# alibaba/EasyRec

Hardware: NVIDIA H100
Metric: samples_per_sec (higher is better)
Workload: dtype f32

## Files before the change

easyrec_b200/_lib.py:

```python
import ctypes
import os

import numpy as np

_HERE = os.path.dirname(os.path.abspath(__file__))
LIB_PATH = os.environ.get('ER_LIB_PATH') or os.path.join(_HERE, 'lib', 'liber_b200.so')

c_i32, c_i64, c_f32 = ctypes.c_int32, ctypes.c_int64, ctypes.c_float
c_vp, c_sz = ctypes.c_void_p, ctypes.c_size_t

SLOT_DTYPE = np.dtype(
    [('num_buckets', '<i8'), ('row_offset', '<i8'), ('seg_begin', '<i4'),
     ('n_seg', '<i4'), ('bucket_mode', '<i4'), ('combiner', '<i4'),
     ('out_buf', '<i4'), ('out_stride', '<i4'), ('out_col', '<i4'),
     ('shard_n', '<i4')],
    align=True)
assert SLOT_DTYPE.itemsize == 48
DENSE_SEG_DTYPE = np.dtype([('offset', '<i8'), ('n', '<i8'), ('l2', '<f4'), ('lr_mult', '<f4')], align=True)
assert DENSE_SEG_DTYPE.itemsize == 24

BUCKET_FARM_DECIMAL, BUCKET_MOD, BUCKET_IDENTITY, BUCKET_NONE, BUCKET_ONE_ROW = 0, 1, 2, 3, 4
COMBINER_SUM, COMBINER_MEAN, COMBINER_SQRTN = 0, 1, 2
COMBINER_UNIT_WEIGHTS = 16
OPT_SGD, OPT_ADAGRAD, OPT_LAZY_ADAM, OPT_ADAM_ROWS, OPT_MOMENTUM = 0, 1, 2, 3, 4
ACT_GELU, ACT_LEAKY_RELU, ACT_ELU, ACT_SELU, ACT_TANH, ACT_SWISH, ACT_SIGMOID = 1, 2, 3, 4, 5, 6, 7
MAX_BUFS = 8
ABI_VERSION = 3
HYPER_LR, HYPER_BETA1_POWER, HYPER_BETA2_POWER, HYPER_GRAD_SCALE, HYPER_N = 0, 1, 2, 3, 4


class ErOpt(ctypes.Structure):
  _fields_ = [('kind', c_i32), ('lr', c_f32), ('beta1', c_f32),
              ('beta2', c_f32), ('eps', c_f32), ('beta1_power', c_f32),
              ('beta2_power', c_f32), ('grad_scale', c_f32), ('hyper_dev', c_vp)]


class ErBnStats(ctypes.Structure):
  _fields_ = [('bias', c_vp), ('save_mean', c_vp), ('save_rstd', c_vp), ('moving_mean', c_vp),
              ('moving_var', c_vp), ('eps', c_f32), ('momentum', c_f32)]


class ErCsvCol(ctypes.Structure):
  _fields_ = [('kind', c_i32), ('width', c_i32), ('inner_sep', ctypes.c_char), ('kv_sep', ctypes.c_char), ('pad_', ctypes.c_char * 6),
              ('default_i64', c_i64), ('default_f32', c_f32), ('pad2_', c_i32), ('default_str', ctypes.c_char_p),
              ('out', c_vp), ('lens', c_vp), ('list_cap', c_i64), ('n_vals', c_i64), ('hash_mod', ctypes.c_uint64), ('weights', c_vp),
              ('step_lens', c_vp)]


ER_OK, ER_ERR_INVALID_ARG, ER_ERR_WORKSPACE, ER_ERR_CUDA, ER_ERR_UNSUPPORTED = range(5)
CSV_SKIP, CSV_I64, CSV_F32, CSV_HASH, CSV_I64_LIST, CSV_F32_VEC, CSV_HASH_LIST, CSV_I64_KV_LIST, CSV_HASH_KV_LIST, CSV_F32_LIST, \
    CSV_I64_STEP_LIST, CSV_HASH_STEP_LIST = range(12)

SIGNATURES = {
    'er_abi_version': (c_i32, []),
# ... 64 lines not shown
    'er_split_cols': (c_i32, [c_vp, c_i32, c_i64, ctypes.POINTER(c_vp), ctypes.POINTER(c_i32),
                              ctypes.POINTER(c_i32), c_i32, c_vp]),
    'er_rowsum_block_fwd': (c_i32, [c_vp, c_i64, c_i32, c_i32, c_vp, c_vp, c_vp, c_sz, c_vp]),
    'er_rowsum_block_bwd': (c_i32, [c_vp, c_vp, c_vp, c_f32, c_i64, c_i32, c_i32, c_vp, c_i32, c_vp]),
    'er_dense1_workspace_bytes': (c_sz, [c_i32]),
    'er_dense1_fwd': (c_i32, [c_vp, c_vp, c_vp, c_i64, c_i32, c_i32, c_vp, c_vp]),
    'er_dense1_bwd': (c_i32, [c_vp, c_vp, c_vp, c_i64, c_i32, c_i32, c_vp, c_i32, c_vp, c_vp, c_vp, c_sz, c_vp]),
    'er_gemm_bn_workspace_bytes': (c_sz, [c_i64, c_i64]),
    'er_gemm_bn': (c_i32, [c_vp, c_i64, c_i32, c_vp, c_i64, c_i32, c_vp, c_i64, c_i64, c_i64, c_i64,
                           ctypes.POINTER(ErBnStats), c_vp, c_sz, c_vp]),
    'er_bn_act_apply': (c_i32, [c_vp, c_vp, c_vp, c_vp, c_vp, c_vp, c_i64, c_i32, c_i32, c_vp, c_vp]),
    'er_fm_block_workspace_bytes': (c_sz, [c_i64]),
    'er_fm_block_fwd': (c_i32, [c_vp, c_i64, c_i32, c_i32, c_i32, c_vp, c_vp, c_vp, c_sz, c_vp]),
    'er_fm_block_bwd': (c_i32, [c_vp, c_vp, c_vp, c_vp, c_f32, c_i64, c_i32, c_i32, c_i32, c_i32, c_vp, c_i32,
                                c_vp]),
    'er_gemm_workspace_bytes': (c_sz, [c_i64, c_i64, c_i64]),
    'er_gemm': (c_i32, [c_vp, c_i64, c_i32, c_vp, c_i64, c_i32, c_vp, c_vp, c_i64, c_i64, c_i64, c_i64,
                        c_vp, c_sz, c_vp]),
    'er_bias_bn_act_fwd': (c_i32, [c_vp, c_vp, c_vp, c_vp, c_vp, c_vp, c_i64,
                                   c_i32, c_f32, c_f32, c_i32, c_i32, c_vp,
                                   c_vp, c_vp, c_vp, c_sz, c_vp]),
    'er_bias_bn_act_bwd': (c_i32, [c_vp, c_vp, c_vp, c_vp, c_vp, c_vp, c_vp,
                                   c_i64, c_i32, c_i32, c_vp, c_vp, c_vp, c_vp,
                                   c_vp, c_sz, c_vp]),
    'er_din_concat_fwd': (c_i32, [c_vp, c_vp, c_i64, c_i32, c_i32, c_vp, c_vp]),
    'er_din_concat_bwd': (c_i32, [c_vp, c_vp, c_vp, c_i64, c_i32, c_i32, c_vp, c_vp, c_i32, c_vp]),
    'er_din_pool_fwd': (c_i32, [c_vp, c_vp, c_vp, c_i64, c_i32, c_i32, c_vp, c_vp, c_vp]),
    'er_din_pool_bwd': (c_i32, [c_vp, c_vp, c_vp, c_vp, c_i64, c_i32, c_i32, c_vp, c_vp, c_i32, c_vp]),
    'er_din_sigmoid_pool_fwd': (c_i32, [c_vp, c_vp, c_vp, c_i64, c_i32, c_i32, c_f32, c_vp, c_vp, c_vp]),
    'er_din_sigmoid_pool_bwd': (c_i32, [c_vp, c_vp, c_vp, c_vp, c_i64, c_i32, c_i32, c_f32, c_vp, c_vp, c_i32,
# ... 54 lines not shown
```

easyrec_b200/csrc/gemm.cu:

```cuda
#include <algorithm>

#include "common.cuh"

namespace er {
namespace gemm {

constexpr int BM = 128, BN = 128, BK = 32;
constexpr int kStages = 3;
constexpr int kPrefetch = 2;
constexpr int kThreads = 256;
constexpr int kTileBytes = 128 * 128;
constexpr int kStageBytes = 4 * kTileBytes;
constexpr int kOutPitch = BN + 8;
constexpr int kStatFloats = 768;
constexpr int kSmemBytes = kStages * kStageBytes + 1024  + kStatFloats * 4 + 16;
static_assert(BM * kOutPitch * 4 <= kStages * kStageBytes, "output tile must fit in the stage ring");

struct Args {
  const float* A;
  const float* B;
  float* C;
  const float* bias;
  float* partials;
  long long lda, ldb, ldc;
  int M, N, K;
  int a_mn, b_mn;
  int k_per_slice;
  int n_slices;
  float* bn_part;
  unsigned int* bn_counter;
  er_bn_stats_t bn;
};

__device__ __forceinline__ uint32_t smem_u32(const void* p) {
  return static_cast<uint32_t>(__cvta_generic_to_shared(p));
}

__device__ __forceinline__ uint64_t make_desc(uint32_t smem_addr) {
  uint64_t d = 0;
  d |= (uint64_t)((smem_addr >> 4) & 0x3fff);
  d |= (uint64_t)1 << 16;
  d |= (uint64_t)(1024 >> 4) << 32;
  d |= (uint64_t)1 << 62;
  return d;
}

__device__ __forceinline__ void wgmma_fence() { asm volatile("wgmma.fence.sync.aligned;" ::: "memory"); }
__device__ __forceinline__ void wgmma_commit() { asm volatile("wgmma.commit_group.sync.aligned;" ::: "memory"); }
template <int N>
__device__ __forceinline__ void wgmma_wait() {
// ... 45 lines not shown
      "%16, %17, %18, %19, %20, %21, %22, %23, %24, %25, %26, %27, %28, %29, %30, %31, "
      "%32, %33, %34, %35, %36, %37, %38, %39, %40, %41, %42, %43, %44, %45, %46, %47, "
      "%48, %49, %50, %51, %52, %53, %54, %55, %56, %57, %58, %59, %60, %61, %62, %63"
      "}, %64, %65, p, 1, 1;\n}\n"
      : "+f"(d[0]), "+f"(d[1]), "+f"(d[2]), "+f"(d[3]), "+f"(d[4]), "+f"(d[5]), "+f"(d[6]), "+f"(d[7]),
        "+f"(d[8]), "+f"(d[9]), "+f"(d[10]), "+f"(d[11]), "+f"(d[12]), "+f"(d[13]), "+f"(d[14]), "+f"(d[15]),
        "+f"(d[16]), "+f"(d[17]), "+f"(d[18]), "+f"(d[19]), "+f"(d[20]), "+f"(d[21]), "+f"(d[22]), "+f"(d[23]),
        "+f"(d[24]), "+f"(d[25]), "+f"(d[26]), "+f"(d[27]), "+f"(d[28]), "+f"(d[29]), "+f"(d[30]), "+f"(d[31]),
        "+f"(d[32]), "+f"(d[33]), "+f"(d[34]), "+f"(d[35]), "+f"(d[36]), "+f"(d[37]), "+f"(d[38]), "+f"(d[39]),
        "+f"(d[40]), "+f"(d[41]), "+f"(d[42]), "+f"(d[43]), "+f"(d[44]), "+f"(d[45]), "+f"(d[46]), "+f"(d[47]),
        "+f"(d[48]), "+f"(d[49]), "+f"(d[50]), "+f"(d[51]), "+f"(d[52]), "+f"(d[53]), "+f"(d[54]), "+f"(d[55]),
        "+f"(d[56]), "+f"(d[57]), "+f"(d[58]), "+f"(d[59]), "+f"(d[60]), "+f"(d[61]), "+f"(d[62]), "+f"(d[63])
      : "l"(da), "l"(db), "r"(1));
}

__device__ __forceinline__ void split_tf32(float x, float& hi, float& lo) {
  uint32_t h = (__float_as_uint(x) + 0x1000u) & 0xffffe000u;
  hi = __uint_as_float(h);
  lo = x - hi;
}

__device__ __forceinline__ float4 mask_chunk(float4 v, int nvalid) {
  if (nvalid < 4) {
    if (nvalid < 1) v.x = 0.f;
    if (nvalid < 2) v.y = 0.f;
    if (nvalid < 3) v.z = 0.f;
    v.w = 0.f;
  }
  return v;
}

struct Pos {
  int mn, k;
};
__device__ __forceinline__ Pos pos_of(int mn_major, int warp, int lane, int j) {
  if (!mn_major) return Pos{(lane >> 3) + 4 * warp + 32 * j, 4 * (lane & 7)};
// ... 35 lines not shown
  }
}

struct Welford {
  float n, mean, m2;
};
__device__ __forceinline__ void wf_merge(Welford& a, const Welford& b) {
  if (b.n == 0.f) return;
  const float n = a.n + b.n;
  const float d = b.mean - a.mean;
  a.mean += d * (b.n / n);
  a.m2 += b.m2 + d * d * (a.n * b.n / n);
  a.n = n;
}

template <int NM>
__global__ void __launch_bounds__(kThreads, 1) gemm_tf32x3_kernel(Args a) {
  constexpr int R = NM / 2;
  extern __shared__ uint8_t smem_raw[];
  const uint32_t raw_u32 = smem_u32(smem_raw);
  const uint32_t smem_base = (raw_u32 + 1023u) & ~1023u;
  uint8_t* base_ptr = smem_raw + (smem_base - raw_u32);
  float* s_stats = reinterpret_cast<float*>(base_ptr + kStages * kStageBytes);
  int* s_flag = reinterpret_cast<int*>(s_stats + kStatFloats);

  const int tid = threadIdx.x, warp = tid >> 5, lane = tid & 31, wg = warp >> 2;
  const int n0 = blockIdx.x * BN, m0 = blockIdx.y * BM;
  const int k_begin = blockIdx.z * a.k_per_slice;
  const int k_end = min(a.K, k_begin + a.k_per_slice);
  const int n_kb = (k_end - k_begin + BK - 1) / BK;

  Pos pa[4], pb[4];
#pragma unroll
  for (int j = 0; j < 4; ++j) {
    pa[j] = pos_of(a.a_mn, warp, lane, j);
    pb[j] = pos_of(a.b_mn, warp, lane, j);
  }
  float4 va[kPrefetch][4], vb[kPrefetch][4];
  auto issue = [&](int kb, float4 (&xa)[4], float4 (&xb)[4]) {
    const int k0 = k_begin + kb * BK;
#pragma unroll
    for (int j = 0; j < 4; ++j) {
      xa[j] = load_pos(a.A, a.lda, a.a_mn, pa[j], m0, a.M, k0, k_end);
      xb[j] = pb[j].mn < NM ? load_pos(a.B, a.ldb, a.b_mn, pb[j], n0, a.N, k0, k_end)
                            : make_float4(0.f, 0.f, 0.f, 0.f);
    }
  };
  auto stage_out = [&](int kb, const float4 (&xa)[4], const float4 (&xb)[4]) {
    const int k0 = k_begin + kb * BK;
    const uint32_t st = smem_base + (uint32_t)(kb % kStages) * kStageBytes;
#pragma unroll
    for (int j = 0; j < 4; ++j) {
      store_pos(st, a.a_mn, pa[j], mask_chunk(xa[j], pos_nvalid(a.a_mn, pa[j], m0, a.M, k0, k_end)));
      if (pb[j].mn < NM)
        store_pos(st + 2 * kTileBytes, a.b_mn, pb[j], mask_chunk(xb[j], pos_nvalid(a.b_mn, pb[j], n0, a.N, k0, k_end)));
    }
  };

  float acc[R], acc2[R];
#pragma unroll
  for (int i = 0; i < R; ++i) acc[i] = acc2[i] = 0.f;

  er_pdl_wait();
#pragma unroll
  for (int u = 0; u < kPrefetch; ++u)
    if (u < n_kb) issue(u, va[u], vb[u]);

  for (int kb0 = 0; kb0 < n_kb; kb0 += kPrefetch) {
#pragma unroll
    for (int u = 0; u < kPrefetch; ++u) {
      const int kb = kb0 + u;
      if (kb < n_kb) {
        stage_out(kb, va[u], vb[u]);
        if (kb + kPrefetch < n_kb) issue(kb + kPrefetch, va[u], vb[u]);
        asm volatile("fence.proxy.async.shared::cta;" ::: "memory");
        __syncthreads();
        const uint32_t st = smem_base + (uint32_t)(kb % kStages) * kStageBytes;
        const uint32_t a_hi = st + (uint32_t)wg * (64u * 128u), b_hi = st + 2 * kTileBytes;
        fence_regs(acc);
        fence_regs(acc2);
        wgmma_fence();
#pragma unroll
        for (int kk = 0; kk < BK / 8; ++kk) {
          const uint64_t ahi = make_desc(a_hi + kk * 32), alo = make_desc(a_hi + kTileBytes + kk * 32);
          const uint64_t bhi = make_desc(b_hi + kk * 32), blo = make_desc(b_hi + kTileBytes + kk * 32);
          wgmma_tf32(acc2, alo, bhi);
          wgmma_tf32(acc2, ahi, blo);
          wgmma_tf32(acc, ahi, bhi);
        }
        wgmma_commit();
        wgmma_wait<1>();
// ... 146 lines not shown

static void plan(int64_t M, int64_t N, int64_t K, int* n_slices, int* k_per_slice) {
  const int64_t tiles = ceil_div(M, BM) * ceil_div(N, BN);
  const int64_t kblocks = ceil_div(K, BK);
  int64_t s = 1;
  if (tiles * 2 <= kSmCount && kblocks >= 16) {
    s = kSmCount / tiles;
    s = std::min<int64_t>(s, kblocks / 8);
    s = std::max<int64_t>(s, 1);
  }
  const int64_t per = ceil_div(kblocks, s);
  *k_per_slice = (int)(per * BK);
  *n_slices = (int)ceil_div(kblocks, per);
}

template <int NM>
static int launch(const Args& a, dim3 grid, cudaStream_t st) {
  static bool attr_set = false;
  if (!attr_set) {
    cudaError_t e = cudaFuncSetAttribute(gemm_tf32x3_kernel<NM>, cudaFuncAttributeMaxDynamicSharedMemorySize,
                                         kSmemBytes);
    if (e != cudaSuccess) return er::fail(ER_ERR_CUDA, std::string("er_gemm: ") + cudaGetErrorString(e));
    attr_set = true;
  }
  er::launch_pdl(gemm_tf32x3_kernel<NM>, grid, dim3(kThreads), (size_t)kSmemBytes, st, a);
  return ER_OK;
}

}
}

extern "C" size_t er_gemm_workspace_bytes(int64_t M, int64_t N, int64_t K) {
  int s, kp;
  er::gemm::plan(M, N, K, &s, &kp);
  return s > 1 ? (size_t)s * (size_t)M * (size_t)N * sizeof(float) : 0;
}

extern "C" size_t er_gemm_bn_workspace_bytes(int64_t M, int64_t N);

static int gemm_impl(const float* A, int64_t lda, int32_t a_mn_major, const float* B, int64_t ldb,
                     int32_t b_mn_major, const float* bias, float* C, int64_t ldc, int64_t M, int64_t N,
                     int64_t K, const er_bn_stats_t* bn, void* ws, size_t ws_bytes, er_stream_t stream) {
  using namespace er::gemm;
  ER_REQUIRE(A && B && C, "null operand");
  ER_REQUIRE(M > 0 && N > 0 && K > 0 && M < (1ll << 31) && N < (1ll << 31) && K < (1ll << 31), "bad shape");
  ER_REQUIRE((lda & 3) == 0 && (ldb & 3) == 0, "operand pitch must be a multiple of 4 floats");
  ER_REQUIRE((reinterpret_cast<uintptr_t>(A) & 15) == 0 && (reinterpret_cast<uintptr_t>(B) & 15) == 0,
             "operands must be 16-byte aligned");
  ER_REQUIRE(lda >= (a_mn_major ? M : K) && ldb >= (b_mn_major ? N : K), "pitch smaller than row");
  ER_REQUIRE(ldc >= N, "ldc < N");
  Args a;
  a.A = A; a.B = B; a.C = C; a.bias = bias;
  a.lda = lda; a.ldb = ldb; a.ldc = ldc;
  a.M = (int)M; a.N = (int)N; a.K = (int)K;
  a.a_mn = a_mn_major ? 1 : 0; a.b_mn = b_mn_major ? 1 : 0;
  plan(M, N, K, &a.n_slices, &a.k_per_slice);
  a.partials = nullptr;
  a.bn_part = nullptr;
  a.bn_counter = nullptr;
  if (a.n_slices > 1) {
    ER_REQUIRE(!bn, "batch-norm statistics need an unsplit K (er_gemm_workspace_bytes(M,N,K) == 0)");
    ER_REQUIRE(ws && ws_bytes >= er_gemm_workspace_bytes(M, N, K), "workspace too small");
    a.partials = static_cast<float*>(ws);
  }
  if (bn) {
    ER_REQUIRE(bn->save_mean && bn->save_rstd, "bn: save_mean / save_rstd missing");
    ER_REQUIRE((bn->moving_mean == nullptr) == (bn->moving_var == nullptr), "bn: moving_mean and moving_var go together");
    ER_REQUIRE(ws && ws_bytes >= er_gemm_bn_workspace_bytes(M, N), "bn workspace too small");
    a.bn = *bn;
    a.bn_counter = static_cast<unsigned int*>(ws);
    a.bn_part = reinterpret_cast<float*>(static_cast<char*>(ws) + 1024);
  }
  cudaStream_t st = er::as_stream(stream);
  dim3 grid((unsigned)er::ceil_div(N, BN), (unsigned)er::ceil_div(M, BM), (unsigned)a.n_slices);
  const int rc = N > 64 ? launch<128>(a, grid, st) : N > 32 ? launch<64>(a, grid, st)
               : N > 16 ? launch<32>(a, grid, st) : launch<16>(a, grid, st);
  if (rc != ER_OK) return rc;
  int launches = 1;
  if (a.n_slices > 1) {
    const long long total = (long long)M * N;
    int blocks = (int)std::min<long long>((total + 255) / 256, 4LL * er::kSmCount);
    er::launch_pdl(splitk_reduce_kernel, dim3(blocks), dim3(256), 0, st, (const float*)a.partials, bias, C,
                   (long long)ldc, (int)M, (int)N, a.n_slices);
    ++launches;
  }
  er::count_launches(launches);
  ER_CUDA_LAUNCH_CHECK();
  return ER_OK;
}

extern "C" int er_gemm(const float* A, int64_t lda, int32_t a_mn_major, const float* B, int64_t ldb,
                       int32_t b_mn_major, const float* bias, float* C, int64_t ldc, int64_t M, int64_t N,
                       int64_t K, void* ws, size_t ws_bytes, er_stream_t stream) {
  return gemm_impl(A, lda, a_mn_major, B, ldb, b_mn_major, bias, C, ldc, M, N, K, nullptr, ws, ws_bytes, stream);
}

extern "C" size_t er_gemm_bn_workspace_bytes(int64_t M, int64_t N) {
  return 1024 + (size_t)er::ceil_div(M, er::gemm::BM) * (size_t)N * 3 * sizeof(float);
}

extern "C" int er_gemm_bn(const float* A, int64_t lda, int32_t a_mn_major, const float* B, int64_t ldb,
                          int32_t b_mn_major, float* C, int64_t ldc, int64_t M, int64_t N, int64_t K,
                          const er_bn_stats_t* bn, void* ws, size_t ws_bytes, er_stream_t stream) {
  if (!bn) return er::fail(ER_ERR_INVALID_ARG, "er_gemm_bn: bn is NULL");
  if (er::ceil_div(N, er::gemm::BN) > 256) return er::fail(ER_ERR_INVALID_ARG, "er_gemm_bn: N too large");
  return gemm_impl(A, lda, a_mn_major, B, ldb, b_mn_major, nullptr, C, ldc, M, N, K, bn, ws, ws_bytes, stream);
}
```

easyrec_b200/kernels.py:

```python
import ctypes

import numpy as np
import torch

from easyrec_b200 import _lib
from easyrec_b200._lib import ErOpt, SLOT_DTYPE, c_vp


def _stream():
  return torch.cuda.current_stream().cuda_stream


def _p(t):
  return None if t is None else t.data_ptr()


def _chk(t, dtype, name):
  if t is None:
    return
  if not t.is_cuda:
    raise _lib.ErError('%s must be a CUDA tensor (no CPU fallback)' % name)
  if t.dtype != dtype:
    raise _lib.ErError('%s must be %s, got %s' % (name, dtype, t.dtype))
  if not t.is_contiguous():
# ... 507 lines not shown
      buf = torch.zeros(t.shape[0], (t.shape[1] + 3) // 4 * 4, dtype=torch.float32, device=t.device)
      buf[:, :t.shape[1]].copy_(t)
      t = buf[:, :t.shape[1]]
    else:
      t = t.contiguous() if not t.is_contiguous() else t.clone()
  raise ValueError('%s: cannot be laid out for er_gemm' % name)


def gemm_ready(t):
  return _gemm_operand(t, 'x')[0]


_gemm_ws = {}


def gemm(a, b, bias=None, out=None):
  lib = _lib.load()
  M, Ka = a.shape
  Kb, N = b.shape
  assert Ka == Kb, (a.shape, b.shape)
  if N < 8 or Ka < 8 or M < 8:
    return gemm_small(a, b, bias, out)
  a, lda, a_unit = _gemm_operand(a, 'a')
  b, ldb, b_unit = _gemm_operand(b, 'b')
  if out is None:
    out = torch.empty(M, N, dtype=torch.float32, device=a.device)
  assert out.stride(1) == 1
  nbytes = lib.er_gemm_workspace_bytes(M, N, Ka)
  ws = None
  if nbytes:
    key = (a.device, torch.cuda.current_stream().cuda_stream if a.is_cuda else 0)
    ws = _gemm_ws.get(key)
    if ws is None or ws.numel() < nbytes:
      ws = torch.empty(nbytes, dtype=torch.uint8, device=a.device)
      _gemm_ws[key] = ws
  _lib.check(lib.er_gemm(_p(a), lda, 0 if a_unit else 1, _p(b), ldb, 1 if b_unit else 0, _p(bias), _p(out),
                         out.stride(0), M, N, Ka, _p(ws), 0 if ws is None else ws.numel(), _stream()), 'er_gemm')
  return out


def gemm_small(a, b, bias=None, out=None):
  lib = _lib.load()
  M, Ka = a.shape
  _, N = b.shape
  for t, name in ((a, 'a'), (b, 'b')):
    if not t.is_cuda or t.dtype != torch.float32:
      raise _lib.ErError('%s must be a CUDA fp32 matrix (no CPU fallback)' % name)
  _chk(bias, torch.float32, 'bias')
  if out is None:
    out = torch.empty(M, N, dtype=torch.float32, device=a.device)
# ... 3 lines not shown
  if nbytes:
    key = (a.device, torch.cuda.current_stream().cuda_stream, 'small')
    ws = _gemm_ws.get(key)
    if ws is None or ws.numel() < nbytes:
      ws = torch.empty(nbytes, dtype=torch.uint8, device=a.device)
      _gemm_ws[key] = ws
  _lib.check(lib.er_gemm_small(_p(a), a.stride(0), a.stride(1), _p(b), b.stride(0), b.stride(1), _p(bias), _p(out),
                               out.stride(0), M, N, Ka, _p(ws), 0 if ws is None else ws.numel(), _stream()),
             'er_gemm_small')
  return out


_gemm_bn_ws = {}


def gemm_bn(a, b, bias, moving_mean, moving_var, eps, momentum):
  lib = _lib.load()
  M, Ka = a.shape
  Kb, N = b.shape
  assert Ka == Kb, (a.shape, b.shape)
  if N < 8 or Ka < 8 or M < 8 or lib.er_gemm_workspace_bytes(M, N, Ka) != 0:
    return None
  a, lda, a_unit = _gemm_operand(a, 'a')
  b, ldb, b_unit = _gemm_operand(b, 'b')
  z = torch.empty(M, N, dtype=torch.float32, device=a.device)
  mean = torch.empty(N, dtype=torch.float32, device=a.device)
  rstd = torch.empty(N, dtype=torch.float32, device=a.device)
  nbytes = lib.er_gemm_bn_workspace_bytes(M, N)
  key = (a.device, torch.cuda.current_stream().cuda_stream if a.is_cuda else 0)
  ws = _gemm_bn_ws.get(key)
  if ws is None or ws.numel() < nbytes:
    ws = torch.zeros(nbytes, dtype=torch.uint8, device=a.device)
    _gemm_bn_ws[key] = ws
  bn = _lib.ErBnStats(_p(bias), _p(mean), _p(rstd), _p(moving_mean), _p(moving_var), eps, momentum)
  _lib.check(lib.er_gemm_bn(_p(a), lda, 0 if a_unit else 1, _p(b), ldb, 1 if b_unit else 0, _p(z), z.stride(0),
                            M, N, Ka, ctypes.byref(bn), _p(ws), ws.numel(), _stream()), 'er_gemm_bn')
  return z, mean, rstd


def bn_act_apply(z, bias, gamma, beta, mean, rstd, relu, y=None):
  lib = _lib.load()
  _chk(z, torch.float32, 'z')
  batch, units = z.shape
  if y is None:
    y = torch.empty_like(z)
  _lib.check(lib.er_bn_act_apply(_p(z), _p(bias), _p(gamma), _p(beta), _p(mean), _p(rstd), batch, units,
                                 1 if relu else 0, _p(y), _stream()), 'er_bn_act_apply')
  return y


def dense_workspace(batch, units, device):
  lib = _lib.load()
# ... 35 lines not shown
```

easyrec_b200/layers.py:

```python
import math
import os

import torch
from torch import nn

from easyrec_b200 import kernels as K

BN_EPS = 1e-3
BN_MOMENTUM = 0.99
_OVERLAP_DW_DX = os.environ.get('ER_OVERLAP_DW_DX', '1') == '1'
_side = {}
_defer = {'on': False, 'dirty': set()}


class defer_dw_join(object):

  def __enter__(self):
    self.prev = _defer['on']
    _defer['on'] = True
    return self

  def __exit__(self, *exc):
    _defer['on'] = self.prev
    if not self.prev:
      for dev in list(_defer['dirty']):
        torch.cuda.current_stream(dev).wait_stream(_side[dev])
      _defer['dirty'].clear()
    return False


def _side_stream(device):
  s = _side.get(device)
  if s is None:
    s = torch.cuda.Stream(device=device)
    _side[device] = s
  return s


class _DenseBNAct(torch.autograd.Function):

  @staticmethod
  def forward(ctx, x, kernel, bias, gamma, beta, moving_mean, moving_var, training, relu, ws):
    x = K.gemm_ready(x)
    ctx.kernel_param = kernel
    if hasattr(kernel, '_er_uses'):
      kernel._er_uses += 1
    fused = None
    if gamma is not None and training:
      fused = K.gemm_bn(x, kernel, bias, moving_mean, moving_var, BN_EPS, BN_MOMENTUM)
    if fused is not None:
      z, mean, rstd = fused
      y = K.bn_act_apply(z, bias, gamma, beta, mean, rstd, relu)
    else:
      z = K.gemm(x, kernel)
      y, mean, rstd = K.bias_bn_act_fwd(z, bias, gamma, beta, moving_mean, moving_var, BN_EPS,
                                        BN_MOMENTUM, training, relu, ws)
    ctx.relu = relu
    ctx.ws = ws
    ctx.has_bn = gamma is not None
    ctx.save_for_backward(x, kernel, bias, gamma, z, y, mean, rstd)
    return y

  @staticmethod
  def backward(ctx, gy):
    x, kernel, bias, gamma, z, y, mean, rstd = ctx.saved_tensors
    gz, gbias, ggamma, gbeta = K.bias_bn_act_bwd(z, bias, gamma, y, gy.contiguous(), mean, rstd,
                                                 ctx.relu, ctx.ws)
    kp = ctx.kernel_param
    dst = getattr(kp, '_er_grad_out', None)
    if dst is not None and getattr(kp, '_er_uses', 2) == 1 and kp.grad is None:
      gk = dst.view_as(dst)
    else:
      gk = torch.empty(x.shape[1], gz.shape[1], dtype=torch.float32, device=x.device)
    if ctx.needs_input_grad[0] and x.is_cuda and _OVERLAP_DW_DX:
      cur = torch.cuda.current_stream()
      side = _side_stream(x.device)
      side.wait_stream(cur)
      with torch.cuda.stream(side):
        K.gemm(x.t(), gz, out=gk)
      gx = K.gemm(gz, kernel.t())
      if _defer['on']:
        gz.record_stream(side)
        x.record_stream(side)
        _defer['dirty'].add(x.device)
      else:
        cur.wait_stream(side)
    else:
      K.gemm(x.t(), gz, out=gk)
      gx = K.gemm(gz, kernel.t()) if ctx.needs_input_grad[0] else None
    return gx, gk, gbias, ggamma, gbeta, None, None, None, None, None


class _Dense1(torch.autograd.Function):

  @staticmethod
  def forward(ctx, x, kernel, bias):
    if x.stride(1) != 1:
      x = x.contiguous()
    ctx.save_for_backward(x, kernel)
    return K.dense1_fwd(x, kernel, bias)

  @staticmethod
  def backward(ctx, gy):
    x, kernel = ctx.saved_tensors
# ... 278 lines not shown
```

easyrec_b200/trainer.py:

```python
import ctypes

import numpy as np
import torch

from easyrec_b200 import _lib
from easyrec_b200 import kernels as K
from easyrec_b200 import layers as L


class FlatDenseOptimizer(object):

  def __init__(self, named_params, kind, lr, l2_of=None, beta1=0.9, beta2=0.999, eps=1e-8,
               adagrad_init=0.1):
    self.names = [n for n, _ in named_params]
    self.params = [p for _, p in named_params]
    dev = self.params[0].device
    sizes = [p.numel() for p in self.params]
    self.sizes = sizes
    total = sum((n + 3) // 4 * 4 for n in sizes)
    self.flat_p = torch.zeros(total, dtype=torch.float32, device=dev)
    self.flat_g = torch.zeros(total, dtype=torch.float32, device=dev)
    off = 0
    segs = np.zeros(len(sizes), dtype=_lib.DENSE_SEG_DTYPE)
    self.grad_views = []
# ... 116 lines not shown
class Trainer(object):

  def __init__(self, model, input_layer, dense_optimizer='adagrad', lr=0.01, lr_fn=None,
               use_cuda_graph=False, world_size=1, beta1=0.9, beta2=0.999, adagrad_init=0.1, dense_lr_fn=None,
               dense_betas=None, clip_norm=0.0):
    self.model = model
    self.input_layer = input_layer
    self.lr = lr
    self.lr_fn = lr_fn or (lambda step: lr)
    named = [(n, p) for n, p in model.named_parameters() if p.requires_grad]
    l2 = getattr(model, 'l2_of', None)
    db1, db2 = dense_betas or (beta1, beta2)
    self.dense_opt = FlatDenseOptimizer(named, dense_optimizer, lr, l2_of=l2, beta1=db1, beta2=db2,
                                        adagrad_init=adagrad_init)
    self.beta1, self.beta2 = beta1, beta2
    self.dense_lr_fn = dense_lr_fn
    if dense_lr_fn is None:
      self.dense_opt.hyper = input_layer.hyper
    self.world = world_size
    self.clip_norm = float(clip_norm or 0.0)
    self.last_grad_norm = None
    self.dp = None
    if world_size > 1:
      from easyrec_b200.distributed import DataParallel
      ep = bool(getattr(input_layer, 'ep', False))
      if self.clip_norm and ep:
        input_layer.ep_hold_updates(True)
      self.dp = DataParallel(input_layer, self.dense_opt, world_size, sparse=not ep)
    dev = str(getattr(input_layer, 'device', 'cpu'))
    self._ep_side = torch.cuda.Stream(device=dev) if (self.dp is not None and not self.dp.sparse and
# ... 8 lines not shown
    self._warm_stream = None
    self._graph = None
    self._step_pending = []
    self._static = None
    self._loss = None
    self._probs = None

  def _set_hyper(self):
    lr = self.lr_fn(self.step)
    self.input_layer.set_optimizer_step(lr, self.step, beta1=self.beta1, beta2=self.beta2)
    if self.dense_lr_fn is not None:
      self.dense_opt.hyper.set(self.dense_lr_fn(self.step), self.step)

  def _segment_compute(self, features, labels, next_features=None):
    self.dense_opt.zero_grad()
    logits = self.model(features)
    if next_features is not None:
      self.input_layer.prefetch_exchange(next_features)
    sw = features.get('sample_weight') if isinstance(features, dict) else None
    if sw is not None:
      loss, probs = self.model.loss(logits, labels, sample_weight=sw)
    else:
      loss, probs = self.model.loss(logits, labels)
    with L.defer_dw_join():
      loss.backward()
    self.dense_opt.gather_grads()
    self._step_pending = list(self.input_layer._pending)
    return loss.detach(), probs

  def _segment_exchange(self):
    if self.dp is not None:
      if not self.dp.sparse:
        if self._ep_side is not None:
          self._ep_side.wait_stream(torch.cuda.current_stream())
        with torch.cuda.stream(self._ep_side):
          self.input_layer.backward_update()
      self.dp.exchange(self._step_pending)
      self.dp.join_presort()

  def _clip_by_global_norm(self):
# ... 109 lines not shown
```

include/er_b200.h:

```cpp
#ifndef ER_B200_H_
#define ER_B200_H_

#include <stddef.h>
#include <stdint.h>

#ifdef __cplusplus
extern "C" {
#endif

#define ER_B200_ABI_VERSION 3

typedef void* er_stream_t;

typedef enum er_status {
  ER_OK = 0,
  ER_ERR_INVALID_ARG = 1,
  ER_ERR_WORKSPACE = 2,
  ER_ERR_CUDA = 3,
  ER_ERR_UNSUPPORTED = 4
} er_status;

typedef enum er_bucket_mode {
  ER_BUCKET_FARM_DECIMAL = 0,
  ER_BUCKET_MOD = 1,
// ... 228 lines not shown
                  er_stream_t stream);

typedef struct {
  const float* bias;
  float* save_mean;
  float* save_rstd;
  float* moving_mean;
  float* moving_var;
  float eps;
  float momentum;
} er_bn_stats_t;
size_t er_gemm_bn_workspace_bytes(int64_t M, int64_t N);
int er_gemm_bn(const float* A, int64_t lda, int32_t a_mn_major, const float* B, int64_t ldb,
               int32_t b_mn_major, float* C, int64_t ldc, int64_t M, int64_t N, int64_t K,
               const er_bn_stats_t* bn, void* ws, size_t ws_bytes, er_stream_t stream);
int er_bn_act_apply(const float* z, const float* bias, const float* gamma, const float* beta,
                    const float* mean, const float* rstd, int64_t batch, int32_t units, int32_t relu,
                    float* y, er_stream_t stream);

int er_sigmoid_ce_fwd_bwd(const float* logits, const float* labels,
                          const float* weights, int64_t batch, float inv_count,
                          float* loss_out, float* probs, float* g_logits,
                          er_stream_t stream);

int er_din_concat_fwd(const float* query, const float* keys, int64_t batch,
                      int32_t seq_len, int32_t dim, float* din_in, er_stream_t stream);
int er_din_concat_bwd(const float* query, const float* keys, const float* g_din_in,
                      int64_t batch, int32_t seq_len, int32_t dim, float* g_query,
                      float* g_keys, int32_t accumulate_gkeys, er_stream_t stream);
int er_din_pool_fwd(const float* scores, const float* keys, const int32_t* lens,
// ... 87 lines not shown
```

Before: 9.935 million.

## Pre-split dense weights into swizzled TF32 hi/lo planes loaded by bulk copy

Once per step, a batched kernel splits each dense tower weight (and its transpose) into TF32 hi/lo planes laid out in the GEMM's swizzled shared-memory tile format. Forward and dX GEMMs then fetch the B operand with cp.async.bulk on mbarriers instead of per-thread loads, splitting and storing. This removes repeated per-CTA B splitting and register staging, and frees registers to deepen A prefetch. It costs an extra split kernel and plane memory every step, and adds mbarrier synchronisation complexity.

```diff
diff --git a/easyrec_b200/_lib.py b/easyrec_b200/_lib.py
--- a/easyrec_b200/_lib.py
+++ b/easyrec_b200/_lib.py
@@ -38,6 +38,11 @@
 class ErBnStats(ctypes.Structure):
   _fields_ = [('bias', c_vp), ('save_mean', c_vp), ('save_rstd', c_vp), ('moving_mean', c_vp),
               ('moving_var', c_vp), ('eps', c_f32), ('momentum', c_f32)]
+
+
+class ErGemmPlane(ctypes.Structure):
+  _fields_ = [('src', c_vp), ('ld_row', c_i64), ('ld_k', c_i64), ('rows', c_i64), ('k', c_i64), ('hi', c_vp),
+              ('lo', c_vp)]
 
 
 class ErCsvCol(ctypes.Structure):
@@ -132,6 +137,10 @@
     'er_fm_block_fwd': (c_i32, [c_vp, c_i64, c_i32, c_i32, c_i32, c_vp, c_vp, c_vp, c_sz, c_vp]),
     'er_fm_block_bwd': (c_i32, [c_vp, c_vp, c_vp, c_vp, c_f32, c_i64, c_i32, c_i32, c_i32, c_i32, c_vp, c_i32,
                                 c_vp]),
+    'er_gemm_plane_floats': (c_sz, [c_i64, c_i64]),
+    'er_gemm_split_planes': (c_i32, [ctypes.POINTER(ErGemmPlane), c_i32, c_vp]),
+    'er_gemm_planes': (c_i32, [c_vp, c_i64, c_i32, c_vp, c_vp, c_vp, c_vp, c_i64, c_i64, c_i64, c_i64,
+                               ctypes.POINTER(ErBnStats), c_vp, c_sz, c_vp]),
     'er_gemm_workspace_bytes': (c_sz, [c_i64, c_i64, c_i64]),
     'er_gemm': (c_i32, [c_vp, c_i64, c_i32, c_vp, c_i64, c_i32, c_vp, c_vp, c_i64, c_i64, c_i64, c_i64,
                         c_vp, c_sz, c_vp]),
diff --git a/easyrec_b200/csrc/gemm.cu b/easyrec_b200/csrc/gemm.cu
--- a/easyrec_b200/csrc/gemm.cu
+++ b/easyrec_b200/csrc/gemm.cu
@@ -1,6 +1,7 @@
 #include <algorithm>
 
 #include "common.cuh"
+#include "tf32_split.cuh"
 
 namespace er {
 namespace gemm {
@@ -8,12 +9,13 @@
 constexpr int BM = 128, BN = 128, BK = 32;
 constexpr int kStages = 3;
 constexpr int kPrefetch = 2;
+constexpr int kPrefetchPre = 3;
 constexpr int kThreads = 256;
 constexpr int kTileBytes = 128 * 128;
 constexpr int kStageBytes = 4 * kTileBytes;
 constexpr int kOutPitch = BN + 8;
 constexpr int kStatFloats = 768;
-constexpr int kSmemBytes = kStages * kStageBytes + 1024  + kStatFloats * 4 + 16;
+constexpr int kSmemBytes = kStages * kStageBytes + 1024  + kStatFloats * 4 + 16 + kStages * 8;
 static_assert(BM * kOutPitch * 4 <= kStages * kStageBytes, "output tile must fit in the stage ring");
 
 struct Args {
@@ -25,6 +27,9 @@
   long long lda, ldb, ldc;
   int M, N, K;
   int a_mn, b_mn;
+  const float* b_hi;
+  const float* b_lo;
+  long long b_tile_floats;
   int k_per_slice;
   int n_slices;
   float* bn_part;
@@ -32,8 +37,30 @@
   er_bn_stats_t bn;
 };
 
+__host__ __device__ constexpr int mma_width(long long n) { return n > 64 ? 128 : n > 32 ? 64 : n > 16 ? 32 : 16; }
+__host__ __device__ constexpr long long plane_tile_floats(long long rows, long long k) {
+  return (k + BK - 1) / BK * mma_width(rows) * BK;
+}
+
 __device__ __forceinline__ uint32_t smem_u32(const void* p) {
   return static_cast<uint32_t>(__cvta_generic_to_shared(p));
+}
+
+__device__ __forceinline__ void mbar_init(uint32_t bar, uint32_t count) {
+  asm volatile("mbarrier.init.shared::cta.b64 [%0], %1;" ::"r"(bar), "r"(count) : "memory");
+}
+__device__ __forceinline__ void mbar_expect_tx(uint32_t bar, uint32_t bytes) {
+  asm volatile("mbarrier.arrive.expect_tx.shared::cta.b64 _, [%0], %1;" ::"r"(bar), "r"(bytes) : "memory");
+}
+__device__ __forceinline__ void mbar_wait(uint32_t bar, uint32_t parity) {
+  asm volatile(
+      "{\n.reg .pred p;\nWAIT_%=:\n"
+      "mbarrier.try_wait.parity.shared::cta.b64 p, [%0], %1;\n"
+      "@!p bra WAIT_%=;\n}\n" ::"r"(bar), "r"(parity) : "memory");
+}
+__device__ __forceinline__ void bulk_g2s(uint32_t dst, const void* src, uint32_t bytes, uint32_t bar) {
+  asm volatile("cp.async.bulk.shared::cluster.global.mbarrier::complete_tx::bytes [%0], [%1], %2, [%3];"
+               ::"r"(dst), "l"(src), "r"(bytes), "r"(bar) : "memory");
 }
 
 __device__ __forceinline__ uint64_t make_desc(uint32_t smem_addr) {
@@ -109,12 +136,6 @@
       : "l"(da), "l"(db), "r"(1));
 }
 
-__device__ __forceinline__ void split_tf32(float x, float& hi, float& lo) {
-  uint32_t h = (__float_as_uint(x) + 0x1000u) & 0xffffe000u;
-  hi = __uint_as_float(h);
-  lo = x - hi;
-}
-
 __device__ __forceinline__ float4 mask_chunk(float4 v, int nvalid) {
   if (nvalid < 4) {
     if (nvalid < 1) v.x = 0.f;
@@ -180,15 +201,17 @@
   a.n = n;
 }
 
-template <int NM>
+template <int NM, bool kPreB>
 __global__ void __launch_bounds__(kThreads, 1) gemm_tf32x3_kernel(Args a) {
   constexpr int R = NM / 2;
+  constexpr int kPf = kPreB ? kPrefetchPre : kPrefetch;
   extern __shared__ uint8_t smem_raw[];
   const uint32_t raw_u32 = smem_u32(smem_raw);
   const uint32_t smem_base = (raw_u32 + 1023u) & ~1023u;
   uint8_t* base_ptr = smem_raw + (smem_base - raw_u32);
   float* s_stats = reinterpret_cast<float*>(base_ptr + kStages * kStageBytes);
   int* s_flag = reinterpret_cast<int*>(s_stats + kStatFloats);
+  const uint32_t s_bar = smem_u32(s_flag + 4);
 
   const int tid = threadIdx.x, warp = tid >> 5, lane = tid & 31, wg = warp >> 2;
   const int n0 = blockIdx.x * BN, m0 = blockIdx.y * BM;
@@ -202,14 +225,15 @@
     pa[j] = pos_of(a.a_mn, warp, lane, j);
     pb[j] = pos_of(a.b_mn, warp, lane, j);
   }
-  float4 va[kPrefetch][4], vb[kPrefetch][4];
+  float4 va[kPf][4], vb[kPreB ? 1 : kPf][4];
   auto issue = [&](int kb, float4 (&xa)[4], float4 (&xb)[4]) {
     const int k0 = k_begin + kb * BK;
 #pragma unroll
     for (int j = 0; j < 4; ++j) {
       xa[j] = load_pos(a.A, a.lda, a.a_mn, pa[j], m0, a.M, k0, k_end);
-      xb[j] = pb[j].mn < NM ? load_pos(a.B, a.ldb, a.b_mn, pb[j], n0, a.N, k0, k_end)
-                            : make_float4(0.f, 0.f, 0.f, 0.f);
+      if constexpr (!kPreB)
+        xb[j] = pb[j].mn < NM ? load_pos(a.B, a.ldb, a.b_mn, pb[j], n0, a.N, k0, k_end)
+                              : make_float4(0.f, 0.f, 0.f, 0.f);
     }
   };
   auto stage_out = [&](int kb, const float4 (&xa)[4], const float4 (&xb)[4]) {
@@ -218,29 +242,50 @@
 #pragma unroll
     for (int j = 0; j < 4; ++j) {
       store_pos(st, a.a_mn, pa[j], mask_chunk(xa[j], pos_nvalid(a.a_mn, pa[j], m0, a.M, k0, k_end)));
-      if (pb[j].mn < NM)
+      if (!kPreB && pb[j].mn < NM)
         store_pos(st + 2 * kTileBytes, a.b_mn, pb[j], mask_chunk(xb[j], pos_nvalid(a.b_mn, pb[j], n0, a.N, k0, k_end)));
     }
   };
+  auto issue_b = [&](int kb) {
+    constexpr uint32_t kPlaneBytes = NM * BK * 4;
+    const uint32_t st = smem_base + (uint32_t)(kb % kStages) * kStageBytes + 2 * kTileBytes;
+    const uint32_t bar = s_bar + 8u * (uint32_t)(kb % kStages);
+    const long long off = (long long)blockIdx.x * a.b_tile_floats + (long long)(k_begin / BK + kb) * (NM * BK);
+    mbar_expect_tx(bar, 2 * kPlaneBytes);
+    bulk_g2s(st, a.b_hi + off, kPlaneBytes, bar);
+    bulk_g2s(st + kTileBytes, a.b_lo + off, kPlaneBytes, bar);
+  };
+  if constexpr (kPreB) {
+    if (tid == 0) {
+      for (int s = 0; s < kStages; ++s) mbar_init(s_bar + 8u * s, 1);
+      asm volatile("fence.mbarrier_init.release.cluster;" ::: "memory");
+    }
+    __syncthreads();
+  }
 
   float acc[R], acc2[R];
 #pragma unroll
   for (int i = 0; i < R; ++i) acc[i] = acc2[i] = 0.f;
 
   er_pdl_wait();
-#pragma unroll
-  for (int u = 0; u < kPrefetch; ++u)
-    if (u < n_kb) issue(u, va[u], vb[u]);
-
-  for (int kb0 = 0; kb0 < n_kb; kb0 += kPrefetch) {
-#pragma unroll
-    for (int u = 0; u < kPrefetch; ++u) {
+  if (kPreB && tid == 0 && n_kb > 0) issue_b(0);
+#pragma unroll
+  for (int u = 0; u < kPf; ++u)
+    if (u < n_kb) issue(u, va[u], vb[kPreB ? 0 : u]);
+
+  for (int kb0 = 0; kb0 < n_kb; kb0 += kPf) {
+#pragma unroll
+    for (int u = 0; u < kPf; ++u) {
       const int kb = kb0 + u;
       if (kb < n_kb) {
-        stage_out(kb, va[u], vb[u]);
-        if (kb + kPrefetch < n_kb) issue(kb + kPrefetch, va[u], vb[u]);
+        stage_out(kb, va[u], vb[kPreB ? 0 : u]);
+        if (kb + kPf < n_kb) issue(kb + kPf, va[u], vb[kPreB ? 0 : u]);
         asm volatile("fence.proxy.async.shared::cta;" ::: "memory");
         __syncthreads();
+        if constexpr (kPreB) {
+          if (tid == 0 && kb + 1 < n_kb) issue_b(kb + 1);
+          mbar_wait(s_bar + 8u * (uint32_t)(kb % kStages), (uint32_t)(kb / kStages) & 1u);
+        }
         const uint32_t st = smem_base + (uint32_t)(kb % kStages) * kStageBytes;
         const uint32_t a_hi = st + (uint32_t)wg * (64u * 128u), b_hi = st + 2 * kTileBytes;
         fence_regs(acc);
@@ -417,17 +462,53 @@
   *n_slices = (int)ceil_div(kblocks, per);
 }
 
-template <int NM>
+template <int NM, bool kPreB>
 static int launch(const Args& a, dim3 grid, cudaStream_t st) {
   static bool attr_set = false;
   if (!attr_set) {
-    cudaError_t e = cudaFuncSetAttribute(gemm_tf32x3_kernel<NM>, cudaFuncAttributeMaxDynamicSharedMemorySize,
+    cudaError_t e = cudaFuncSetAttribute(gemm_tf32x3_kernel<NM, kPreB>, cudaFuncAttributeMaxDynamicSharedMemorySize,
                                          kSmemBytes);
     if (e != cudaSuccess) return er::fail(ER_ERR_CUDA, std::string("er_gemm: ") + cudaGetErrorString(e));
     attr_set = true;
   }
-  er::launch_pdl(gemm_tf32x3_kernel<NM>, grid, dim3(kThreads), (size_t)kSmemBytes, st, a);
+  er::launch_pdl(gemm_tf32x3_kernel<NM, kPreB>, grid, dim3(kThreads), (size_t)kSmemBytes, st, a);
   return ER_OK;
+}
+template <bool kPreB>
+static int launch_width(const Args& a, dim3 grid, cudaStream_t st) {
+  switch (mma_width(a.N)) {
+    case 128: return launch<128, kPreB>(a, grid, st);
+    case 64: return launch<64, kPreB>(a, grid, st);
+    case 32: return launch<32, kPreB>(a, grid, st);
+    default: return launch<16, kPreB>(a, grid, st);
+  }
+}
+
+constexpr int kMaxPlaneJobs = 32;
+struct PlaneJobs {
+  er_gemm_plane_t j[kMaxPlaneJobs];
+};
+__global__ void split_planes_kernel(PlaneJobs jobs) {
+  const er_gemm_plane_t p = jobs.j[blockIdx.y];
+  const int nm = mma_width(p.rows);
+  const long long n_kb = (p.k + BK - 1) / BK;
+  const long long chunks = (p.rows + BN - 1) / BN * n_kb * nm * (BK / 4);
+  er_pdl_wait();
+  for (long long i = (long long)blockIdx.x * blockDim.x + threadIdx.x; i < chunks; i += (long long)gridDim.x * blockDim.x) {
+    const int c = (int)(i & 7);
+    const long long rk = i >> 3;
+    const int r = (int)(rk % nm);
+    const long long tkb = rk / nm;
+    const long long row = tkb / n_kb * nm + r, k0 = tkb % n_kb * BK + 4 * (c ^ (r & 7));
+    float v[4], hi[4], lo[4];
+#pragma unroll
+    for (int e = 0; e < 4; ++e) {
+      v[e] = row < p.rows && k0 + e < p.k ? p.src[row * p.ld_row + (k0 + e) * p.ld_k] : 0.f;
+      split_tf32(v[e], hi[e], lo[e]);
+    }
+    reinterpret_cast<float4*>(p.hi)[i] = make_float4(hi[0], hi[1], hi[2], hi[3]);
+    reinterpret_cast<float4*>(p.lo)[i] = make_float4(lo[0], lo[1], lo[2], lo[3]);
+  }
 }
 
 }
@@ -442,18 +523,22 @@
 extern "C" size_t er_gemm_bn_workspace_bytes(int64_t M, int64_t N);
 
 static int gemm_impl(const float* A, int64_t lda, int32_t a_mn_major, const float* B, int64_t ldb,
-                     int32_t b_mn_major, const float* bias, float* C, int64_t ldc, int64_t M, int64_t N,
-                     int64_t K, const er_bn_stats_t* bn, void* ws, size_t ws_bytes, er_stream_t stream) {
+                     int32_t b_mn_major, const float* b_hi, const float* b_lo, const float* bias, float* C,
+                     int64_t ldc, int64_t M, int64_t N, int64_t K, const er_bn_stats_t* bn, void* ws,
+                     size_t ws_bytes, er_stream_t stream) {
   using namespace er::gemm;
-  ER_REQUIRE(A && B && C, "null operand");
+  const bool pre_b = B == nullptr;
+  ER_REQUIRE(A && C && (pre_b ? b_hi && b_lo : true), "null operand");
   ER_REQUIRE(M > 0 && N > 0 && K > 0 && M < (1ll << 31) && N < (1ll << 31) && K < (1ll << 31), "bad shape");
-  ER_REQUIRE((lda & 3) == 0 && (ldb & 3) == 0, "operand pitch must be a multiple of 4 floats");
-  ER_REQUIRE((reinterpret_cast<uintptr_t>(A) & 15) == 0 && (reinterpret_cast<uintptr_t>(B) & 15) == 0,
+  ER_REQUIRE((lda & 3) == 0 && (pre_b || (ldb & 3) == 0), "operand pitch must be a multiple of 4 floats");
+  ER_REQUIRE((reinterpret_cast<uintptr_t>(A) & 15) == 0 && (reinterpret_cast<uintptr_t>(B) & 15) == 0 &&
+                 (reinterpret_cast<uintptr_t>(b_hi) & 15) == 0 && (reinterpret_cast<uintptr_t>(b_lo) & 15) == 0,
              "operands must be 16-byte aligned");
-  ER_REQUIRE(lda >= (a_mn_major ? M : K) && ldb >= (b_mn_major ? N : K), "pitch smaller than row");
+  ER_REQUIRE(lda >= (a_mn_major ? M : K) && (pre_b || ldb >= (b_mn_major ? N : K)), "pitch smaller than row");
   ER_REQUIRE(ldc >= N, "ldc < N");
   Args a;
   a.A = A; a.B = B; a.C = C; a.bias = bias;
+  a.b_hi = b_hi; a.b_lo = b_lo; a.b_tile_floats = plane_tile_floats(N, K);
   a.lda = lda; a.ldb = ldb; a.ldc = ldc;
   a.M = (int)M; a.N = (int)N; a.K = (int)K;
   a.a_mn = a_mn_major ? 1 : 0; a.b_mn = b_mn_major ? 1 : 0;
@@ -476,8 +561,7 @@
   }
   cudaStream_t st = er::as_stream(stream);
   dim3 grid((unsigned)er::ceil_div(N, BN), (unsigned)er::ceil_div(M, BM), (unsigned)a.n_slices);
-  const int rc = N > 64 ? launch<128>(a, grid, st) : N > 32 ? launch<64>(a, grid, st)
-               : N > 16 ? launch<32>(a, grid, st) : launch<16>(a, grid, st);
+  const int rc = pre_b ? launch_width<true>(a, grid, st) : launch_width<false>(a, grid, st);
   if (rc != ER_OK) return rc;
   int launches = 1;
   if (a.n_slices > 1) {
@@ -495,7 +579,9 @@
 extern "C" int er_gemm(const float* A, int64_t lda, int32_t a_mn_major, const float* B, int64_t ldb,
                        int32_t b_mn_major, const float* bias, float* C, int64_t ldc, int64_t M, int64_t N,
                        int64_t K, void* ws, size_t ws_bytes, er_stream_t stream) {
-  return gemm_impl(A, lda, a_mn_major, B, ldb, b_mn_major, bias, C, ldc, M, N, K, nullptr, ws, ws_bytes, stream);
+  ER_REQUIRE(B, "null operand");
+  return gemm_impl(A, lda, a_mn_major, B, ldb, b_mn_major, nullptr, nullptr, bias, C, ldc, M, N, K, nullptr, ws,
+                   ws_bytes, stream);
 }
 
 extern "C" size_t er_gemm_bn_workspace_bytes(int64_t M, int64_t N) {
@@ -507,5 +593,47 @@
                           const er_bn_stats_t* bn, void* ws, size_t ws_bytes, er_stream_t stream) {
   if (!bn) return er::fail(ER_ERR_INVALID_ARG, "er_gemm_bn: bn is NULL");
   if (er::ceil_div(N, er::gemm::BN) > 256) return er::fail(ER_ERR_INVALID_ARG, "er_gemm_bn: N too large");
-  return gemm_impl(A, lda, a_mn_major, B, ldb, b_mn_major, nullptr, C, ldc, M, N, K, bn, ws, ws_bytes, stream);
-}
+  ER_REQUIRE(B, "null operand");
+  return gemm_impl(A, lda, a_mn_major, B, ldb, b_mn_major, nullptr, nullptr, nullptr, C, ldc, M, N, K, bn, ws,
+                   ws_bytes, stream);
+}
+
+extern "C" size_t er_gemm_plane_floats(int64_t rows, int64_t K) {
+  if (rows <= 0 || K <= 0) return 0;
+  return (size_t)er::ceil_div(rows, (int64_t)er::gemm::BN) * (size_t)er::gemm::plane_tile_floats(rows, K);
+}
+
+extern "C" int er_gemm_split_planes(const er_gemm_plane_t* planes, int32_t n, er_stream_t stream) {
+  using namespace er::gemm;
+  ER_REQUIRE(n >= 0 && (n == 0 || planes), "bad plane list");
+  cudaStream_t st = er::as_stream(stream);
+  int launches = 0;
+  for (int i0 = 0; i0 < n; i0 += kMaxPlaneJobs) {
+    PlaneJobs jobs;
+    const int cnt = std::min(kMaxPlaneJobs, n - i0);
+    long long max_chunks = 0;
+    for (int i = 0; i < cnt; ++i) {
+      const er_gemm_plane_t& p = planes[i0 + i];
+      ER_REQUIRE(p.src && p.hi && p.lo, "null plane pointer");
+      ER_REQUIRE(p.rows > 0 && p.k > 0 && p.rows < (1ll << 31) && p.k < (1ll << 31), "bad plane shape");
+      ER_REQUIRE((reinterpret_cast<uintptr_t>(p.hi) & 15) == 0 && (reinterpret_cast<uintptr_t>(p.lo) & 15) == 0,
+                 "planes must be 16-byte aligned");
+      jobs.j[i] = p;
+      max_chunks = std::max<long long>(max_chunks, (long long)er_gemm_plane_floats(p.rows, p.k) / 4);
+    }
+    const int blocks = (int)std::min<long long>((max_chunks + 255) / 256, 2LL * er::kSmCount);
+    er::launch_pdl(split_planes_kernel, dim3(blocks, cnt), dim3(256), 0, st, jobs);
+    ++launches;
+  }
+  er::count_launches(launches);
+  ER_CUDA_LAUNCH_CHECK();
+  return ER_OK;
+}
+
+extern "C" int er_gemm_planes(const float* A, int64_t lda, int32_t a_mn_major, const float* b_hi, const float* b_lo,
+                              const float* bias, float* C, int64_t ldc, int64_t M, int64_t N, int64_t K,
+                              const er_bn_stats_t* bn, void* ws, size_t ws_bytes, er_stream_t stream) {
+  if (bn && bias) return er::fail(ER_ERR_INVALID_ARG, "er_gemm_planes: with bn the bias goes in bn->bias");
+  if (bn && er::ceil_div(N, er::gemm::BN) > 256) return er::fail(ER_ERR_INVALID_ARG, "er_gemm_planes: N too large");
+  return gemm_impl(A, lda, a_mn_major, nullptr, 0, 0, b_hi, b_lo, bias, C, ldc, M, N, K, bn, ws, ws_bytes, stream);
+}
diff --git a/easyrec_b200/csrc/tf32_split.cuh b/easyrec_b200/csrc/tf32_split.cuh
--- /dev/null
+++ b/easyrec_b200/csrc/tf32_split.cuh
@@ -0,0 +1,25 @@
+#pragma once
+#include <stdint.h>
+#include <string.h>
+
+#ifdef __CUDACC__
+#define ER_SPLIT_HD __host__ __device__ __forceinline__
+#else
+#define ER_SPLIT_HD inline
+#endif
+
+namespace er {
+
+ER_SPLIT_HD void split_tf32(float x, float& hi, float& lo) {
+#ifdef __CUDA_ARCH__
+  hi = __uint_as_float((__float_as_uint(x) + 0x1000u) & 0xffffe000u);
+#else
+  uint32_t u;
+  memcpy(&u, &x, 4);
+  u = (u + 0x1000u) & 0xffffe000u;
+  memcpy(&hi, &u, 4);
+#endif
+  lo = x - hi;
+}
+
+}
diff --git a/easyrec_b200/kernels.py b/easyrec_b200/kernels.py
--- a/easyrec_b200/kernels.py
+++ b/easyrec_b200/kernels.py
@@ -545,7 +545,7 @@
 _gemm_ws = {}
 
 
-def gemm(a, b, bias=None, out=None):
+def gemm(a, b, bias=None, out=None, planes=None):
   lib = _lib.load()
   M, Ka = a.shape
   Kb, N = b.shape
@@ -553,7 +553,8 @@
   if N < 8 or Ka < 8 or M < 8:
     return gemm_small(a, b, bias, out)
   a, lda, a_unit = _gemm_operand(a, 'a')
-  b, ldb, b_unit = _gemm_operand(b, 'b')
+  if planes is None:
+    b, ldb, b_unit = _gemm_operand(b, 'b')
   if out is None:
     out = torch.empty(M, N, dtype=torch.float32, device=a.device)
   assert out.stride(1) == 1
@@ -565,6 +566,11 @@
     if ws is None or ws.numel() < nbytes:
       ws = torch.empty(nbytes, dtype=torch.uint8, device=a.device)
       _gemm_ws[key] = ws
+  if planes is not None:
+    _lib.check(lib.er_gemm_planes(_p(a), lda, 0 if a_unit else 1, _p(planes[0]), _p(planes[1]), _p(bias), _p(out),
+                                  out.stride(0), M, N, Ka, None, _p(ws), 0 if ws is None else ws.numel(), _stream()),
+               'er_gemm_planes')
+    return out
   _lib.check(lib.er_gemm(_p(a), lda, 0 if a_unit else 1, _p(b), ldb, 1 if b_unit else 0, _p(bias), _p(out),
                          out.stride(0), M, N, Ka, _p(ws), 0 if ws is None else ws.numel(), _stream()), 'er_gemm')
   return out
@@ -598,7 +604,7 @@
 _gemm_bn_ws = {}
 
 
-def gemm_bn(a, b, bias, moving_mean, moving_var, eps, momentum):
+def gemm_bn(a, b, bias, moving_mean, moving_var, eps, momentum, planes=None):
   lib = _lib.load()
   M, Ka = a.shape
   Kb, N = b.shape
@@ -606,7 +612,8 @@
   if N < 8 or Ka < 8 or M < 8 or lib.er_gemm_workspace_bytes(M, N, Ka) != 0:
     return None
   a, lda, a_unit = _gemm_operand(a, 'a')
-  b, ldb, b_unit = _gemm_operand(b, 'b')
+  if planes is None:
+    b, ldb, b_unit = _gemm_operand(b, 'b')
   z = torch.empty(M, N, dtype=torch.float32, device=a.device)
   mean = torch.empty(N, dtype=torch.float32, device=a.device)
   rstd = torch.empty(N, dtype=torch.float32, device=a.device)
@@ -617,9 +624,44 @@
     ws = torch.zeros(nbytes, dtype=torch.uint8, device=a.device)
     _gemm_bn_ws[key] = ws
   bn = _lib.ErBnStats(_p(bias), _p(mean), _p(rstd), _p(moving_mean), _p(moving_var), eps, momentum)
+  if planes is not None:
+    _lib.check(lib.er_gemm_planes(_p(a), lda, 0 if a_unit else 1, _p(planes[0]), _p(planes[1]), None, _p(z),
+                                  z.stride(0), M, N, Ka, ctypes.byref(bn), _p(ws), ws.numel(), _stream()),
+               'er_gemm_planes')
+    return z, mean, rstd
   _lib.check(lib.er_gemm_bn(_p(a), lda, 0 if a_unit else 1, _p(b), ldb, 1 if b_unit else 0, _p(z), z.stride(0),
                             M, N, Ka, ctypes.byref(bn), _p(ws), ws.numel(), _stream()), 'er_gemm_bn')
   return z, mean, rstd
+
+
+class DensePlanes(object):
+
+  def __init__(self, kernels, device):
+    lib = _lib.load()
+    self.kernels = list(kernels)
+    for w in self.kernels:
+      assert w.dim() == 2 and w.dtype == torch.float32 and w.is_cuda and w.is_contiguous()
+    jobs = []
+    for w in self.kernels:
+      n_in, n_out = w.shape
+      jobs.append((n_out, n_in, 1, n_out))
+      jobs.append((n_in, n_out, n_out, 1))
+    sizes = [int(lib.er_gemm_plane_floats(rows, k)) for rows, k, _, _ in jobs]
+    self.buf = torch.empty(2 * sum(sizes), dtype=torch.float32, device=device)
+    self.planes = []
+    self.jobs = (_lib.ErGemmPlane * len(jobs))()
+    off = 0
+    for i, ((rows, k, ld_row, ld_k), n) in enumerate(zip(jobs, sizes)):
+      hi, lo = self.buf[off:off + n], self.buf[off + n:off + 2 * n]
+      off += 2 * n
+      self.planes.append((hi, lo))
+      self.jobs[i] = _lib.ErGemmPlane(_p(self.kernels[i // 2]), ld_row, ld_k, rows, k, _p(hi), _p(lo))
+
+  def refresh(self):
+    _lib.check(_lib.load().er_gemm_split_planes(self.jobs, len(self.planes), _stream()), 'er_gemm_split_planes')
+
+  def view(self, i, transposed):
+    return self.planes[2 * i + (1 if transposed else 0)]
 
 
 def bn_act_apply(z, bias, gamma, beta, mean, rstd, relu, y=None):
diff --git a/easyrec_b200/layers.py b/easyrec_b200/layers.py
--- a/easyrec_b200/layers.py
+++ b/easyrec_b200/layers.py
@@ -11,6 +11,7 @@
 _OVERLAP_DW_DX = os.environ.get('ER_OVERLAP_DW_DX', '1') == '1'
 _side = {}
 _defer = {'on': False, 'dirty': set()}
+_planes = {'on': None}
 
 
 class defer_dw_join(object):
@@ -29,6 +30,35 @@
     return False
 
 
+def tower_kernels(model):
+  return [m.kernel for m in model.modules()
+          if isinstance(m, DenseLayer) and m.kernel.requires_grad and min(m.kernel.shape) >= 8]
+
+
+class use_planes(object):
+
+  def __init__(self, planes):
+    self.planes = planes
+    self.index = {id(w): i for i, w in enumerate(planes.kernels)} if planes is not None else {}
+
+  def __enter__(self):
+    self.prev = _planes['on']
+    _planes['on'] = self
+    return self
+
+  def __exit__(self, *exc):
+    _planes['on'] = self.prev
+    return False
+
+
+def _kernel_planes(kernel):
+  ctx = _planes['on']
+  i = ctx.index.get(id(kernel)) if ctx is not None else None
+  if i is None:
+    return None, None
+  return ctx.planes.view(i, False), ctx.planes.view(i, True)
+
+
 def _side_stream(device):
   s = _side.get(device)
   if s is None:
@@ -45,14 +75,16 @@
     ctx.kernel_param = kernel
     if hasattr(kernel, '_er_uses'):
       kernel._er_uses += 1
+    fwd_planes, ctx.dx_planes = _kernel_planes(kernel)
+    pk = {} if fwd_planes is None else {'planes': fwd_planes}
     fused = None
     if gamma is not None and training:
-      fused = K.gemm_bn(x, kernel, bias, moving_mean, moving_var, BN_EPS, BN_MOMENTUM)
+      fused = K.gemm_bn(x, kernel, bias, moving_mean, moving_var, BN_EPS, BN_MOMENTUM, **pk)
     if fused is not None:
       z, mean, rstd = fused
       y = K.bn_act_apply(z, bias, gamma, beta, mean, rstd, relu)
     else:
-      z = K.gemm(x, kernel)
+      z = K.gemm(x, kernel, **pk)
       y, mean, rstd = K.bias_bn_act_fwd(z, bias, gamma, beta, moving_mean, moving_var, BN_EPS,
                                         BN_MOMENTUM, training, relu, ws)
     ctx.relu = relu
@@ -72,13 +104,14 @@
       gk = dst.view_as(dst)
     else:
       gk = torch.empty(x.shape[1], gz.shape[1], dtype=torch.float32, device=x.device)
+    pk = {} if ctx.dx_planes is None else {'planes': ctx.dx_planes}
     if ctx.needs_input_grad[0] and x.is_cuda and _OVERLAP_DW_DX:
       cur = torch.cuda.current_stream()
       side = _side_stream(x.device)
       side.wait_stream(cur)
       with torch.cuda.stream(side):
         K.gemm(x.t(), gz, out=gk)
-      gx = K.gemm(gz, kernel.t())
+      gx = K.gemm(gz, kernel.t(), **pk)
       if _defer['on']:
         gz.record_stream(side)
         x.record_stream(side)
@@ -87,7 +120,7 @@
         cur.wait_stream(side)
     else:
       K.gemm(x.t(), gz, out=gk)
-      gx = K.gemm(gz, kernel.t()) if ctx.needs_input_grad[0] else None
+      gx = K.gemm(gz, kernel.t(), **pk) if ctx.needs_input_grad[0] else None
     return gx, gk, gbias, ggamma, gbeta, None, None, None, None, None
 
 
diff --git a/easyrec_b200/trainer.py b/easyrec_b200/trainer.py
--- a/easyrec_b200/trainer.py
+++ b/easyrec_b200/trainer.py
@@ -154,6 +154,8 @@
     self.dense_opt = FlatDenseOptimizer(named, dense_optimizer, lr, l2_of=l2, beta1=db1, beta2=db2,
                                         adagrad_init=adagrad_init)
     self.beta1, self.beta2 = beta1, beta2
+    kernels = L.tower_kernels(model)
+    self.planes = K.DensePlanes(kernels, kernels[0].device) if kernels and kernels[0].is_cuda else None
     self.dense_lr_fn = dense_lr_fn
     if dense_lr_fn is None:
       self.dense_opt.hyper = input_layer.hyper
@@ -192,16 +194,19 @@
 
   def _segment_compute(self, features, labels, next_features=None):
     self.dense_opt.zero_grad()
-    logits = self.model(features)
-    if next_features is not None:
-      self.input_layer.prefetch_exchange(next_features)
-    sw = features.get('sample_weight') if isinstance(features, dict) else None
-    if sw is not None:
-      loss, probs = self.model.loss(logits, labels, sample_weight=sw)
-    else:
-      loss, probs = self.model.loss(logits, labels)
-    with L.defer_dw_join():
-      loss.backward()
+    if self.planes is not None:
+      self.planes.refresh()
+    with L.use_planes(self.planes):
+      logits = self.model(features)
+      if next_features is not None:
+        self.input_layer.prefetch_exchange(next_features)
+      sw = features.get('sample_weight') if isinstance(features, dict) else None
+      if sw is not None:
+        loss, probs = self.model.loss(logits, labels, sample_weight=sw)
+      else:
+        loss, probs = self.model.loss(logits, labels)
+      with L.defer_dw_join():
+        loss.backward()
     self.dense_opt.gather_grads()
     self._step_pending = list(self.input_layer._pending)
     return loss.detach(), probs
diff --git a/include/er_b200.h b/include/er_b200.h
--- a/include/er_b200.h
+++ b/include/er_b200.h
@@ -266,6 +266,18 @@
 int er_gemm_bn(const float* A, int64_t lda, int32_t a_mn_major, const float* B, int64_t ldb,
                int32_t b_mn_major, float* C, int64_t ldc, int64_t M, int64_t N, int64_t K,
                const er_bn_stats_t* bn, void* ws, size_t ws_bytes, er_stream_t stream);
+typedef struct {
+  const float* src;
+  int64_t ld_row, ld_k;
+  int64_t rows, k;
+  float* hi;
+  float* lo;
+} er_gemm_plane_t;
+size_t er_gemm_plane_floats(int64_t rows, int64_t K);
+int er_gemm_split_planes(const er_gemm_plane_t* planes, int32_t n, er_stream_t stream);
+int er_gemm_planes(const float* A, int64_t lda, int32_t a_mn_major, const float* b_hi, const float* b_lo,
+                   const float* bias, float* C, int64_t ldc, int64_t M, int64_t N, int64_t K,
+                   const er_bn_stats_t* bn, void* ws, size_t ws_bytes, er_stream_t stream);
 int er_bn_act_apply(const float* z, const float* bias, const float* gamma, const float* beta,
                     const float* mean, const float* rstd, int64_t batch, int32_t units, int32_t relu,
                     float* y, er_stream_t stream);
```

Result: faster. 10.76 million (median of 6 runs) (+8.3%).
